# laomao0/BIN

Hardware: AMD Instinct MI355X
Metric: interpolated frames/sec at 1280x720 (higher is better)
Workload: dtype f16x3 (fp16 hi+lo pairs = 22-bit significands, 3 MFMA products, f32 accumulate; fp32-class: 1e-6 vs the fp32 reference); 1 GPU; Adobe240 test_blur 1280x720 inference, batch=1 per GPU (6-frame window padded to 768x1344 by the test.py rule), window-sharded; precision=f16x3, streams=1, pipelined_steps=False, four_call_schedule=False, parity=max-abs <= 2e-5 (f16x3) vs the fp32 reference (tests/)

## Files before the change

bin_amd/csrc/binhip_conv_common.h:

```cpp
#pragma once
#include "binhip_internal.h"
#include <type_traits>
#ifndef BINHIP_TIMELINE
#define BINHIP_TIMELINE 0
#endif

typedef _Float16 half8 __attribute__((ext_vector_type(8)));
typedef _Float16 half4 __attribute__((ext_vector_type(4)));
typedef float floatx16 __attribute__((ext_vector_type(16)));
typedef float floatx4 __attribute__((ext_vector_type(4)));
typedef __attribute__((address_space(3))) void lds_void_t;
typedef unsigned u32x4 __attribute__((ext_vector_type(4)));

int bh_launch_upnet_ring(const void* x_hi, const void* x_lo, const float* wvar, const float* bvar, float* out, const float* const* images,
                         int nimg, int N, int H, int W, int cin, hipStream_t s);
int bh_upnet_gsub(const float* g, int N, int H, int W, const float* scale, void* y_hi, void* y_lo, void* status, hipStream_t s);
int bh_upnet_ring_dgrad(const float* g, const float* wvar, const float* scale, void* gx_hi, void* gx_lo, void* status, int N, int H, int W,
                        int cin, hipStream_t s);
int bh_upnet_ring_wgrad(const float* g, const void* x_hi, const void* x_lo, float* dwvar, float* dbvar, int N, int H, int W, int cin,
                        int accumulate, hipStream_t s);
struct ConvKArgs {
    const _Float16* x_hi;
    const _Float16* x_lo;
    const _Float16* w_hi;
    const _Float16* w_lo;
    const float* bias;
    _Float16* y_hi;
    _Float16* y_lo;
    const _Float16* r_hi;
    const _Float16* r_lo;
    const _Float16* r2_hi;
    const _Float16* r2_lo;
    const _Float16* m_hi;
    float* out_f32;
    const float* img[5];
    unsigned* flags;
    long long group_stride;
    int N, H, W;
// ... 559 lines not shown
```

bin_amd/csrc/binhip_fused.h:

```cpp
#pragma once
#include "binhip_conv_common.h"

struct TailKArgs {
    const _Float16 *x_hi, *x_lo;
    const _Float16 *wc_hi, *wc_lo;
    const _Float16 *wl_hi, *wl_lo;
    const float *bc, *bl;
    _Float16 *y_hi, *y_lo;
    _Float16 *o3_hi, *o3_lo;
    unsigned* flags;
    int N, H, W, tiles_x, tiles_y, wt;
#if BINHIP_TIMELINE
    void* tl;
    unsigned tl_launch, tl_base;
#endif
};

int bh_launch_tail_x3(const TailKArgs& a, hipStream_t s);
```

bin_amd/csrc/binhip_fused.hip:

```cpp
#include "binhip_conv_common.h"

#include "binhip_fused.h"

template <int NT, int NBUF>
struct TailCfg {
    static constexpr int R = 2, NW = 8, TH = 16, PH = 18, PW = 34;
    static constexpr int PP = 20, CWP = 9, LWP = 3;
    static constexpr int NPL = (NT == 3) ? 2 : 1;
    static constexpr int PLANE_BYTES = (PP + CWP + LWP) * 1024;
    static constexpr int BUF_BYTES = NPL * PLANE_BYTES;
    static constexpr int TAILW_BYTES = NPL * 2 * LWP * 1024;
    static constexpr int LDS_BYTES = NBUF * BUF_BYTES + TAILW_BYTES + 1024;
    static constexpr int NPJ = 3, NCJ = 2, NLJ = 1;
    static constexpr int PS = NPL * (NPJ + NCJ + NLJ);
    static constexpr int NCHUNK = 12;
    static_assert(LDS_BYTES <= 160 * 1024, "LDS budget");
    static_assert(NBUF <= 2 || (NBUF - 2) * PS <= 63, "vmcnt immediate range");
    static_assert(NW * R * 32 * 2 * 32 * NPL <= BUF_BYTES, "o3 staging tile must fit one stage buffer");
};

template <class C>
__device__ __forceinline__ void tail_issue(const TailKArgs& a, char* smem, int c, int buf, int wave, int lane,
                                           const unsigned (&voff)[C::NPJ], const ConvTile& t) {
    char* dummy = smem + (C::LDS_BYTES - 1024);
#pragma unroll
    for (int pl = 0; pl < C::NPL; ++pl) {
        char* lds = smem + buf * C::BUF_BYTES + pl * C::PLANE_BYTES;
// ... 4 lines not shown
            const bool real = i < C::PP;
            __builtin_amdgcn_raw_ptr_buffer_load_lds(rs, (lds_void_t*)(real ? lds + i * 1024 : dummy), 16,
                                                     real ? voff[j] : 0x80000000u, 0, 0, 0);
        }
        __amdgpu_buffer_rsrc_t ws = __builtin_amdgcn_make_buffer_rsrc(
            (void*)((pl ? a.wc_lo : a.wc_hi) + (long long)c * (9 * 32 * 16)), 0, 9 * 1024, 0x00020000);
#pragma unroll
        for (int j = 0; j < C::NCJ; ++j) {
            const int i = wave + C::NW * j;
            const bool real = i < C::CWP;
            __builtin_amdgcn_raw_ptr_buffer_load_lds(ws, (lds_void_t*)(real ? lds + (C::PP + i) * 1024 : dummy), 16,
                                                     real ? (unsigned)(lane * 16) : 0x80000000u, real ? i * 1024 : 0, 0, 0);
        }
        __amdgpu_buffer_rsrc_t ls = __builtin_amdgcn_make_buffer_rsrc(
            (void*)((pl ? a.wl_lo : a.wl_hi) + (long long)c * (96 * 16)), 0, 3 * 1024, 0x00020000);
        {
            const bool real = wave < C::LWP;
            __builtin_amdgcn_raw_ptr_buffer_load_lds(ls, (lds_void_t*)(real ? lds + (C::PP + C::CWP + wave) * 1024 : dummy), 16,
                                                     real ? (unsigned)(lane * 16) : 0x80000000u, real ? wave * 1024 : 0, 0, 0);
        }
    }
}

template <int NT, int NBUF>
__global__ void __launch_bounds__(512)
rdb_tail_kernel(const TailKArgs a, const float* __restrict__ bias_c, const float* __restrict__ bias_l) {
    using C = TailCfg<NT, NBUF>;
    extern __shared__ __attribute__((aligned(16))) char smem[];
    const int tid = threadIdx.x;
    const int lane = tid & 63;
    const int wave = __builtin_amdgcn_readfirstlane(tid >> 6);
    const int n = lane & 31, kg = lane >> 5;

    const ConvTile t = tile_decode<C::TH>(a, 1);
    const int img = t.img, tx0 = t.tx0, ty0 = t.ty0;
    const int H = a.H, W = a.W;
    const long long plane_elems = t.plane_elems;

    unsigned voff[C::NPJ];
#pragma unroll
    for (int j = 0; j < C::NPJ; ++j) {
        const int i = wave + C::NW * j;
        const int q = i * 64 + lane;
        const int p = q >> 1, s = q & 1;
        const int py = p / C::PW, px = p - py * C::PW;
        const int gy = ty0 + py - 1, gx = tx0 + px - 1;
        const int cg = s ^ ((p >> 3) & 1);
        const bool ok = (p < C::PH * C::PW) && gy >= 0 && gy < H && gx >= 0 && gx < W;
        voff[j] = ok ? (unsigned)((((long long)img * H + gy) * W + gx) * 32 + cg * 16) : 0x80000000u;
    }
// ... 48 lines not shown
#pragma unroll
            for (int rr = 0; rr < C::R + 2; ++rr) {
                const int p = b_lane_p + rr * C::PW + dx;
                const int off = p * 32 + ((kg ^ ((p >> 3) & 1)) << 4);
                Bh[rr] = ld8(pb + off);
                if constexpr (NT == 3) Bl[rr] = ld8(pb + C::PLANE_BYTES + off);
            }
#pragma unroll
            for (int dy = 0; dy < 3; ++dy) {
                const int off = ((dy * 3 + dx) * 32) * 32 + a_lane_off;
                const half8 Ah = ld8(wb + off);
                half8 Al;
                if constexpr (NT == 3) Al = ld8(wb + C::PLANE_BYTES + off);
#pragma unroll
                for (int r = 0; r < C::R; ++r) {
                    if constexpr (NT == 3) {
                        accc[r] = mfma_32x32x16(Al, Bh[r + dy], accc[r]);
                        accc[r] = mfma_32x32x16(Ah, Bl[r + dy], accc[r]);
                    }
                    accc[r] = mfma_32x32x16(Ah, Bh[r + dy], accc[r]);
                }
            }
            if (dx == 1) {
                if (st < 6) {
#pragma unroll
                    for (int r = 0; r < C::R; ++r) {
#pragma unroll
                        for (int mt = 0; mt < 3; ++mt) {
                            if (mt == (st >> 1)) {
                                accl[mt][r] = mfma_32x32x16(ident[st & 1], Bh[r + 1], accl[mt][r]);
                                if constexpr (NT == 3)
                                    accl[mt][r] = mfma_32x32x16(ident[st & 1], Bl[r + 1], accl[mt][r]);
                            }
                        }
                    }
                }
#pragma unroll
                for (int mt = 0; mt < 3; ++mt) {
                    const int off = (mt * 32) * 32 + a_lane_off;
                    const half8 Ah = ld8(lb + off);
                    half8 Al;
                    if constexpr (NT == 3) Al = ld8(lb + C::PLANE_BYTES + off);
#pragma unroll
                    for (int r = 0; r < C::R; ++r) {
                        if constexpr (NT == 3) {
                            accl[mt][r] = mfma_32x32x16(Al, Bh[r + 1], accl[mt][r]);
                            accl[mt][r] = mfma_32x32x16(Ah, Bl[r + 1], accl[mt][r]);
// ... 108 lines not shown
                    split_pair(v[0], v[1], sat, hv[ge].u[0], lv[ge].u[0]);
                    split_pair(v[2], v[3], sat, hv[ge].u[1], lv[ge].u[1]);
                }
#pragma unroll
                for (int k = 0; k < 2; ++k) {
                    auto sw = __builtin_amdgcn_permlane32_swap(hv[0].u[k], hv[1].u[k], false, false);
                    hv[0].u[k] = sw[0]; hv[1].u[k] = sw[1];
                    if constexpr (NT == 3) {
                        auto sl = __builtin_amdgcn_permlane32_swap(lv[0].u[k], lv[1].u[k], false, false);
                        lv[0].u[k] = sl[0]; lv[1].u[k] = sl[1];
                    }
                }
                if (ok) {
                    store16(a.y_hi, o_slot, make_uint4(hv[0].u[0], hv[0].u[1], hv[1].u[0], hv[1].u[1]), a.wt);
                    if constexpr (NT == 3)
                        store16(a.y_lo, o_slot, make_uint4(lv[0].u[0], lv[0].u[1], lv[1].u[0], lv[1].u[1]), a.wt);
                }
            }
        }
    }
    if (a.flags && __builtin_amdgcn_ballot_w64(sat != 0) != 0 && lane == 0) atomicOr(a.flags, BINHIP_FLAG_SATURATED);
}

template <int NT, int NBUF>
static int launch_tail(const TailKArgs& a0, hipStream_t s) {
    using C = TailCfg<NT, NBUF>;
    static std::atomic<unsigned long long> lds_set{0};
    if (int rc = bh_set_max_lds(&rdb_tail_kernel<NT, NBUF>, C::LDS_BYTES, lds_set)) return rc;
    TailKArgs a = a0;
    rdb_tail_kernel<NT, NBUF><<<dim3(set_tiles<C>(a)), dim3(512), C::LDS_BYTES, s>>>(a, a.bc, a.bl);
    BH_CHECK_LAUNCH();
    return 0;
}

extern "C" {

int binhip_rdb_tail_fwd(int N, int H, int W, int nterms, const void* blk_hi, const void* blk_lo, const void* wc_hi,
                        const void* wc_lo, const float* bias_c, const void* wl_hi, const void* wl_lo, const float* bias_l,
                        void* y_hi, void* y_lo, int store_o3, void* status, void* stream) {
    if (!blk_hi || !wc_hi || !wl_hi || !bias_c || !bias_l || !y_hi) return BINHIP_E_ARG;
    if (nterms != 1 && nterms != 3) return BINHIP_E_ARG;
    if (nterms == 3 && (!blk_lo || !wc_lo || !wl_lo || !y_lo)) return BINHIP_E_ARG;
    if (N <= 0 || H <= 0 || W <= 0) return BINHIP_E_SHAPE;
    if ((long long)N * H * W >= (1ll << 26)) return BINHIP_E_SHAPE;
    TailKArgs a;
    a.x_hi = (const _Float16*)blk_hi; a.x_lo = (const _Float16*)blk_lo;
    a.wc_hi = (const _Float16*)wc_hi; a.wc_lo = (const _Float16*)wc_lo;
    a.wl_hi = (const _Float16*)wl_hi; a.wl_lo = (const _Float16*)wl_lo;
    a.bc = bias_c; a.bl = bias_l;
    a.y_hi = (_Float16*)y_hi; a.y_lo = (_Float16*)y_lo;
    const long long plane = (long long)N * H * W * 16;
    a.o3_hi = store_o3 ? (_Float16*)blk_hi + 12 * plane : nullptr;
    a.o3_lo = (store_o3 && nterms == 3) ? (_Float16*)blk_lo + 12 * plane : nullptr;
    a.flags = (unsigned*)status;
    a.N = N; a.H = H; a.W = W; a.tiles_x = a.tiles_y = 0;
    a.wt = (6 * plane * 2 < (1ll << 32) - 64) ? 1 : 0;
    hipStream_t s = (hipStream_t)stream;
    if (nterms == 1) return launch_tail<1, 2>(a, s);
    return bh_launch_tail_x3(a, s);
}

}
```

bin_amd/csrc/binhip_fused_x3.hip:

```cpp
#include "binhip_fused.h"
#include <type_traits>

namespace {

struct TX {
    static constexpr int R = 2, NW = 4, TH = 8, PH = 10, PW = 34;
    static constexpr int PP = (PH * PW * 2 + 63) / 64;
    static constexpr int CWP = 9, LWP = 3;
    static constexpr int PATCH_BYTES = PP * 1024;
    static constexpr int WPL = (CWP + LWP) * 1024;
    static constexpr int WBUF_BYTES = 2 * WPL;
    static constexpr int W_OFF = 2 * PATCH_BYTES;
    static constexpr int LDS_BYTES = W_OFF + 2 * WBUF_BYTES;
    static constexpr int NCHUNK = 12;
    static constexpr int NPJ = (PP + NW - 1) / NW;
    static constexpr int TAILW_OFF = W_OFF;
    static_assert(2 * LDS_BYTES <= 160 * 1024, "two workgroups per CU");
};

__device__ __forceinline__ void tx_issue_patch(const TailKArgs& a, char* smem, int c, int pl, int wave, const unsigned* voff,
                                               const ConvTile& t) {
    __amdgpu_buffer_rsrc_t rs = patch_plane(a, c, pl, t);
    char* lds = smem + pl * TX::PATCH_BYTES;
#pragma unroll
// ... 99 lines not shown
#pragma unroll
                for (int r = 0; r < R; ++r)
                    accc[r] = mfma_32x32x16(Al[s & 1], B[set][r + k], accc[r]);
            }
#pragma unroll
            for (int r = 0; r < R; ++r)
                accc[r] = mfma_32x32x16(Ah[s & 1], B[set][r + k], accc[r]);
        } else {
            if constexpr (HI) {
#pragma unroll
                for (int r = 0; r < R; ++r)
                    accl[k][r] = mfma_32x32x16(Al[s & 1], B[1][r + 1], accl[k][r]);
            }
#pragma unroll
            for (int r = 0; r < R; ++r)
                accl[k][r] = mfma_32x32x16(Ah[s & 1], B[1][r + 1], accl[k][r]);
        }
        __builtin_amdgcn_sched_barrier(0);
    }
#pragma unroll
    for (int r = 0; r < R; ++r) carry[r] = B[1][r + 1];
}

__global__ void __launch_bounds__(256) __attribute__((amdgpu_waves_per_eu(2, 2)))
rdb_tail_x3_kernel(const TailKArgs a, const float* __restrict__ bias_c, const float* __restrict__ bias_l) {
    extern __shared__ __attribute__((aligned(16))) char smem[];
    BH_TL_DECL;
    BH_TL_BEGIN();
    const int tid = threadIdx.x;
    const int lane = tid & 63;
    const int wave = __builtin_amdgcn_readfirstlane(tid >> 6);
    const int n = lane & 31, kg = lane >> 5;

    const ConvTile t = tile_decode<TX::TH>(a, 1);
    const int img = t.img, tx0 = t.tx0, ty0 = t.ty0;
    const int H = a.H, W = a.W;
    const long long plane_elems = t.plane_elems;
    unsigned voff[TX::NPJ];
    patch_offsets<TX, 1>(voff, t, H, W, wave, lane);

    floatx16 accc[TX::R];
    floatx16 accl[3][TX::R];
#pragma unroll
    for (int r = 0; r < TX::R; ++r)
#pragma unroll
        for (int e = 0; e < 16; ++e) {
// ... 7 lines not shown
    tx_issue_weights(a, smem, 0, 0, wave, lane);
    tx_issue_patch(a, smem, 0, 0, wave, voff, t);
    half8 carry[TX::R];
    auto chunk = [&](const int c, auto res_hi, auto res_lo) __attribute__((always_inline)) {
        constexpr int RH = decltype(res_hi)::value, RL = decltype(res_lo)::value;
        const char* wb = smem + TX::W_OFF + (c & 1) * TX::WBUF_BYTES;
        wait_vmcnt<0>();
        __builtin_amdgcn_s_barrier();
        __builtin_amdgcn_sched_barrier(0);
#if BINHIP_TIMELINE
        if (c == 0) BH_TL_STAMP(1);
#endif
        tx_issue_patch(a, smem, c, 1, wave, voff, t);
        if (c + 1 < TX::NCHUNK) tx_issue_weights(a, smem, c + 1, (c + 1) & 1, wave, lane);
        else tx_issue_tailw(a, smem, wave, lane);
        tx_compute<true, RH>(smem, wb, a_lane_off, b_lane_off, accc, accl, carry);
        wait_vmcnt<0>();
        __builtin_amdgcn_s_barrier();
        __builtin_amdgcn_sched_barrier(0);
        if (c + 1 < TX::NCHUNK) tx_issue_patch(a, smem, c + 1, 0, wave, voff, t);
        tx_compute<false, RL>(smem + TX::PATCH_BYTES, wb, a_lane_off, b_lane_off, accc, accl, carry);
    };
    using std::integral_constant;
    chunk(0, integral_constant<int, -1>{}, integral_constant<int, 0>{});
    chunk(1, integral_constant<int, 0>{}, integral_constant<int, 1>{});
    chunk(2, integral_constant<int, 1>{}, integral_constant<int, 2>{});
    chunk(3, integral_constant<int, 2>{}, integral_constant<int, 3>{});
    chunk(4, integral_constant<int, 3>{}, integral_constant<int, 4>{});
    chunk(5, integral_constant<int, 4>{}, integral_constant<int, 5>{});
    chunk(6, integral_constant<int, 5>{}, integral_constant<int, -1>{});
    for (int c = 7; c < TX::NCHUNK; ++c) chunk(c, integral_constant<int, -1>{}, integral_constant<int, -1>{});
    wait_vmcnt<0>();
    __builtin_amdgcn_s_barrier();
    __builtin_amdgcn_sched_barrier(0);

    __builtin_amdgcn_s_setprio(0);
    const int gx = tx0 + n;
    union H4 { half4 h; unsigned u[2]; };
    union H8 { half8 h; unsigned u[4]; };
    unsigned sat = 0;
    half8 Bh[2][TX::R], Bl[2][TX::R];
#pragma unroll
    for (int r = 0; r < TX::R; ++r) {
        const int gy = ty0 + wave * TX::R + r;
        const bool ok = (gy < H) && (gx < W);
#pragma unroll
        for (int gp = 0; gp < 2; ++gp) {
            H4 hv[2], lv[2];
#pragma unroll
            for (int ge = 0; ge < 2; ++ge) {
                const int g = 2 * gp + ge;
                float b8[8];
#pragma unroll
                for (int j = 0; j < 8; ++j) b8[j] = bias_c[8 * g + j];
// ... 34 lines not shown
            for (int r = 0; r < TX::R; ++r) {
                accl[mt][r] = mfma_32x32x16(Al, Bh[t][r], accl[mt][r]);
                accl[mt][r] = mfma_32x32x16(Ah, Bh[t][r], accl[mt][r]);
                accl[mt][r] = mfma_32x32x16(Ah, Bl[t][r], accl[mt][r]);
            }
        }
    }
    if (a.flags && __builtin_amdgcn_ballot_w64(sat != 0) != 0 && lane == 0) atomicOr(a.flags, BINHIP_FLAG_SATURATED);
    BH_TL_STAMP(2);

    ConvKArgs e;
    e.bias = a.bl; e.y_hi = a.y_hi; e.y_lo = a.y_lo;
    e.r_hi = e.r_lo = e.r2_hi = e.r2_lo = e.m_hi = nullptr;
    e.flags = a.flags;
    e.N = a.N; e.H = H; e.W = W;
    e.relu = 0; e.has_res = 0; e.cout = 96; e.wt = a.wt;
    e.och_limit = 6; e.res_chunks = 0; e.mask_from = 0; e.y_cpg = 0; e.y_cpg_inv = 0; e.y_group_stride = 0; e.y_unshuf = 0;
    conv_epilogue<3, TX::R, 3, BINHIP_EPI_PLANES, false>(e, bias_l, accl, img, ty0 + wave * TX::R, tx0, 0, true, n, kg, plane_elems);
    BH_TL_FINISH(a, blockIdx.x);
}

}

int bh_launch_tail_x3(const TailKArgs& a0, hipStream_t s) {
    static std::atomic<unsigned long long> lds_set{0};
    if (int rc = bh_set_max_lds(&rdb_tail_x3_kernel, TX::LDS_BYTES, lds_set)) return rc;
    TailKArgs a = a0;
    const unsigned grid = set_tiles<TX>(a);
#if BINHIP_TIMELINE
    a.tl = bh_tl_reserve(grid, &a.tl_base);
    a.tl_launch = (2u << 24) | (g_bh_tl_serial.fetch_add(1) & 0xFFFFFFu);
#endif
    rdb_tail_x3_kernel<<<dim3(grid), dim3(256), TX::LDS_BYTES, s>>>(a, a.bc, a.bl);
    BH_CHECK_LAUNCH();
    return 0;
}
```

bin_amd/csrc/binhip_plan.hip:

```cpp
#include "binhip_conv_common.h"

namespace {

struct Shp {
    int G0, D, C, G;
    int c0, cg, cb;
    int L;
    bool stage4;
};
bool resolve_shape(const BinRdnShape* s, Shp* o) {
    Shp h;
    const bool dflt = !s || (s->G0 == 0 && s->D == 0 && s->C == 0 && s->G == 0);
    h.G0 = dflt ? 96 : s->G0; h.D = dflt ? 12 : s->D; h.C = dflt ? 4 : s->C; h.G = dflt ? 32 : s->G;
    if (h.G0 < 32 || h.G0 > 256 || h.G0 % 32 || h.G < 32 || h.G > 128 || h.G % 32) return false;
    if (h.C < 1 || h.C > BINHIP_RDN_MAX_CONVS || h.D < 1 || h.D > 20) return false;
    h.c0 = h.G0 / 16; h.cg = h.G / 16; h.cb = h.c0 + h.C * h.cg;
    h.L = 2 + h.D * (h.C + 1) + 4;
    if (h.L > BINHIP_RDN_MAX_LAYERS) return false;
    h.stage4 = (h.G0 == 96 && h.C == 4 && h.G == 32);
    *o = h;
    return true;
}
inline int layer_conv(const Shp& sh, int d, int c) { return 2 + d * (sh.C + 1) + c; }

// ... 106 lines not shown
        if (l.ks == 1 && l.epi == BINHIP_EPI_PLANES && c.d.W > 32 && c.d.W % 32 == 0) { c.d.H *= c.d.W / 32; c.d.W = 32; }
        if (l.layer == 0 && l.ks == 5 && (12 * nin) % 16 >= 1 && (12 * nin) % 16 <= 8) c.d.reserved = BINHIP_CONV_HALF_LAST_CHUNK;
        c.x_hi = A.hi(l.x); c.x_lo = A.lo(l.x);
        c.w_hi = p->w_hi[l.layer]; c.w_lo = p->w_lo[l.layer]; c.bias = p->bias[l.layer];
        c.r_hi = A.hi(l.res); c.r_lo = A.lo(l.res);
        c.y_hi = A.hi(l.y); c.y_lo = A.lo(l.y);
        c.status = p->status; c.prof = p->profiler;
        if (l.epi == BINHIP_EPI_FINAL || l.epi == BINHIP_EPI_FINAL_SUBPIX) {
            c.y_f32 = out; c.d.n_images = nin;
            for (int i = 0; i < nin; ++i) c.images[i] = inputs[i];
        }
        return c;
    };
    auto conv = [&](const Conv& l) -> int { return bh_launch_conv(mk(l), s); };
    const bool rdb3 = (p->reserved & BINHIP_PLAN_RDB3) && nt == 3 && sh.stage4;
    unsigned* sync_words = (unsigned*)(A.base + w.sync);
    const int cus = binhip_device_cus();
    if (rdb3) {
        hipError_t me = hipMemsetAsync(sync_words, 0, (size_t)(32 + 2 * (size_t)w.tiles) * 4, s);
        if (me != hipSuccess) return (int)me;
    }
    const int64_t P = w.P;
    const int G0 = sh.G0, G = sh.G, C = sh.C, D = sh.D, c0 = sh.c0, cg = sh.cg, cb = sh.cb;
    if ((rc = conv({.layer = 0, .ks = 5, .cin_chunks = w.kc0, .cout = G0, .x = w.x0, .y = w.f1}))) return rc;
    if ((rc = conv({.layer = 1, .cin_chunks = c0, .cout = G0, .x = w.f1, .y = w.blk}))) return rc;
    for (int d = 0; d < D; ++d) {
        const Planes b = w.blk.sub((int64_t)d * cb * P), b_next = b.sub(cb * P);
        auto dense = [&](int c) -> Conv {
            return {.layer = layer_conv(sh, d, c), .cin_chunks = c0 + cg * c, .cout = G, .relu = 1, .x = b, .y = b.sub((c0 + cg * c) * P)};
        };
        const bool fuse = sh.stage4 && !(p->reserved & BINHIP_PLAN_NO_FUSE);
        bool done3 = false;
        if (rdb3 && fuse) {
            ConvKArgs ka[3];
            bool ok3 = true;
            for (int c = 0; c < 3 && ok3; ++c) {
                if ((rc = bh_prepare_conv(mk(dense(c)), &ka[c]))) return rc;
                ok3 = ok3 && ka[c].wt;
            }
            if (ok3) {
                rc = bh_launch_rdb3_x3(ka, sync_words + 32, (unsigned)(d + 1), cus, s);
                if (rc == 0) done3 = true;
                else if (rc != BINHIP_E_SHAPE) return rc;
            }
        }
        for (int c = 0; c < (fuse ? C - 1 : C) && !done3; ++c) if ((rc = conv(dense(c)))) return rc;
        if (fuse) {
            const int L3 = layer_conv(sh, d, 3), LF = layer_conv(sh, d, 4);
            if ((rc = binhip_rdb_tail_fwd(N, h, ww, nt, A.hi(b), A.lo(b), p->w_hi[L3], p->w_lo[L3], p->bias[L3], p->w_hi[LF], p->w_lo[LF], p->bias[LF],
                                          A.hi(b_next), A.lo(b_next), (p->reserved & BINHIP_PLAN_KEEP_ACTS) ? 1 : 0, p->status, stream)))
                return rc;
        } else if ((rc = conv({.layer = layer_conv(sh, d, C), .ks = 1, .cin_chunks = cb, .cout = G0, .x = b, .y = b_next, .res = b})))
            return rc;
    }
    const int LG = sh.L - 4;
    if ((rc = conv({.layer = LG, .ks = 1, .cin_chunks = D * c0, .cout = G0, .x = w.blk.sub(cb * P), .x_cpg = c0, .x_group_stride = cb * P, .y = w.g0})))
        return rc;
    if ((rc = conv({.layer = LG + 1, .cin_chunks = c0, .cout = G0, .x = w.g0, .y = w.g1, .res = w.f1}))) return rc;
    const bool fused_up = (p->reserved & BINHIP_PLAN_FUSED_UPNET) &&
                          (!(p->reserved & BINHIP_PLAN_KEEP_ACTS) || (p->reserved & BINHIP_PLAN_FUSED_UPNET_TRAIN)) &&
                          sh.L + 1 < BINHIP_RDN_MAX_LAYERS && p->w_hi[sh.L] && (nt == 1 || p->w_lo[sh.L]) && p->bias[sh.L] &&
                          p->w_hi[sh.L + 1] && p->bias[sh.L + 1];
    const bool fold = (p->reserved & BINHIP_PLAN_UPNET_FOLD) != 0;
    if (fused_up) {
        if ((rc = conv({.layer = sh.L, .ks = 5, .cin_chunks = c0, .cout = 12, .cout_pad = 32, .epi = BINHIP_EPI_FINAL_SUBPIX, .x = w.g1,
                        .reserved = fold ? BINHIP_CONV_UPNET_FOLD : 0})))
            return rc;
        return bh_launch_upnet_ring(A.hi(w.g1), A.lo(w.g1), (const float*)p->w_hi[sh.L + 1], p->bias[sh.L + 1], out, inputs, nin, N, h, ww,
                                    G0, s);
    }
    if ((rc = conv({.layer = LG + 2, .cin_chunks = c0, .cout = 256, .epi = BINHIP_EPI_SHUFFLE, .x = w.g1, .y = w.u}))) return rc;
    return conv({.layer = LG + 3, .cin_chunks = 4, .cout = 3, .cout_pad = 32, .epi = BINHIP_EPI_FINAL, .H = H, .W = W, .x = w.u});
}

}

namespace {

struct Bws {
// ... 242 lines not shown
```

bin_amd/models/archs/RDN.py:

```python
import ctypes as C
import os

import torch
import torch.nn as nn
import torch.nn.init as weight_init

from ... import ops
from ...rdn_plan import RdnWeights, rdn_forward

PRECISIONS = {"f16": 1, "f16x3": 3}


def default_precision():
    p = os.environ.get("BIN_AMD_PRECISION", "f16x3")
    if p not in PRECISIONS:
        raise ValueError(f"BIN_AMD_PRECISION must be one of {sorted(PRECISIONS)}, got {p!r}")
    return p


class _nullctx:
    def __enter__(self):
        return self

    def __exit__(self, *a):
# ... 77 lines not shown
    N_INPUTS = 0

    def __init__(self, G0=64, D=6, C=4, G=32):
        super().__init__()
        from ...rdn_plan import check_shape
        self.shape = check_shape((G0, D, C, G))
        self.G0, self.D, self.C, self.G = G0, D, C, G
        kSize = 3
        self.SFENet1 = nn.Conv2d(12 * self.N_INPUTS, G0, 5, padding=2, stride=1)
        self.SFENet2 = nn.Conv2d(G0, G0, kSize, padding=1, stride=1)
        self.RDBs = nn.ModuleList([RDB(growRate0=G0, growRate=G, nConvLayers=C) for _ in range(D)])
        self.GFF = nn.Sequential(nn.Conv2d(D * G0, G0, 1, padding=0, stride=1),
                                 nn.Conv2d(G0, G0, kSize, padding=1, stride=1))
        self.UPNet = nn.Sequential(nn.Conv2d(G0, 256, kSize, padding=1, stride=1), nn.PixelShuffle(2),
                                   nn.Conv2d(64, 3, kSize, padding=1, stride=1))
        self.precision = None
        from ...autograd import default_backward_precision, default_wgrad_side_stream
        from ...rdn_plan import default_plan_flags
        self.backward_precision = default_backward_precision()
        self._direct_grads = False
        self.allow_f16_training = False
        self.wgrad_side_stream = default_wgrad_side_stream()
        self.plan_flags = default_plan_flags()
        self.profiler = None
        self.bwd_profiler = None
        self.debug_hook = None
        self._wcache = None
        self._wgen = 0

    def direct_param_grads(self, on=True):
        return _DirectParamGrads([self], on)

    def _weights_key(self, nterms):
        params = list(self.parameters())
        return (nterms, str(params[0].device), self._wgen, tuple((p.data_ptr(), p._version) for p in params))

    def invalidate_kernel_weights(self):
        self._wgen += 1

    def kernel_weights(self, nterms):
        key = self._weights_key(nterms)
        if self._wcache is None or self._wcache[0] != key:
            with torch.no_grad():
                self._wcache = (key, RdnWeights(dict(self.named_parameters()), self.N_INPUTS, nterms, shape=self.shape))
        return self._wcache[1]

    def _run(self, *frames):
        if len(frames) != self.N_INPUTS:
            raise TypeError(f"{type(self).__name__}.forward takes {self.N_INPUTS} frames")
        if not all(f.is_cuda for f in frames):
            raise RuntimeError("bin_amd: RDN sub-networks run on a HIP device only (no CPU fallback; see oracle/)")
        with torch.cuda.device(frames[0].device):
            if torch.is_grad_enabled() and (any(f.requires_grad for f in frames) or
                                             any(p.requires_grad for p in self.parameters())):
                from ...autograd import rdn_apply
                return rdn_apply(self, frames)
            nterms = PRECISIONS[self.precision or default_precision()]
            return rdn_forward(self.kernel_weights(nterms), list(frames), flags=self.plan_flags, profiler=self.profiler)


class RDN_residual_interp_2_input(_RDNBase):
    N_INPUTS = 2

    def forward(self, B0, B1):
        return self._run(B0, B1)


class RDN_residual_interp_2_1_input(_RDNBase):
    N_INPUTS = 3

    def forward(self, I0, I1, I2):
        return self._run(I0, I1, I2)


class RDN_residual_interp_4_1_input(_RDNBase):
    N_INPUTS = 5

    def forward(self, B0, B1, B2, B3, B4):
        return self._run(B0, B1, B2, B3, B4)


# ... 34 lines not shown
            I5 = self.model2_2(I4, I4, I6)
            I7 = self.model2_3(I6, I6, I8)
            I4pp = self.model3_1(I3, B3, I3, I5, B5)
            I6pp = self.model3_2(I5, B5, I5, I7, B7)
            I5ppp = self.model4_1(I4, I4, I4pp, I6pp, I6)
        self.I2_prime, self.I4_prime, self.I6_prime, self.I8_prime = I2, I4, I6, I8
        self.I3_prime, self.I5_prime, self.I7_prime = I3, I5, I7
        self.I4_prime_prime, self.I6_prime_prime, self.I5_prime_prime = I4pp, I6pp, I5ppp
        return I2, I4, I6, I8, I3, I5, I7, I4pp, I6pp, I5ppp


class RDN_residual_interp_5_input_ConvLSTM_L(nn.Module):

    def __init__(self, modelType="lstm"):
        super().__init__()
        self.modelType = modelType
        self.clstm_4_prime = ConvLSTMCell(3, 3)
        self.clstm_6_prime = ConvLSTMCell(3, 3)
        self.clstm_8_prime = ConvLSTMCell(3, 3)
        self.clstm_5_prime_prime = ConvLSTMCell(3, 3)
        self.clstm_7_prime_prime = ConvLSTMCell(3, 3)
        self.clstm_6_prime_prime_prime = ConvLSTMCell(3, 3)
        self.model = RDN_residual_interp_5_input(lstm=True, GO=96, D=12)
        self.prev_state = None
        self.hidden_state = None
        self.reuse_schedule = True
        self.precision = None
        self.n_streams = int(os.environ["BIN_AMD_STREAMS"]) if os.environ.get("BIN_AMD_STREAMS") else None
        self.four_calls = os.environ.get("BIN_AMD_FOUR_CALLS", "1") != "0"
        self.four_calls_infer = os.environ.get("BIN_AMD_INFER_FOUR", "auto")
        self._streams = None

    def set_precision(self, precision):
        if precision is not None and precision not in PRECISIONS:
            raise ValueError(f"precision must be one of {sorted(PRECISIONS)}")
        self.precision = precision
        for m in self.modules():
            if isinstance(m, _RDNBase):
                m.precision = precision
        return self

    def rdn_modules(self):
        seen, out = set(), []
        for m in self.modules():
            if isinstance(m, _RDNBase) and id(m) not in seen:
                seen.add(id(m))
# ... 80 lines not shown
def _forward_streams(self, B, stage1_cache=None, input_events=None):
    from ...rdn_plan import rdn_forward, workspace
    from ... import _lib as L
    dev = B[0].device
    main = torch.cuda.current_stream(dev)
    ns = self.resolved_streams()
    if ns == 1:
        streams = [main]
    else:
        if self._streams is None or len(self._streams) != ns or self._streams[0].device != dev:
            self._streams = [torch.cuda.Stream(device=dev) for _ in range(ns)]
        streams = self._streams
    m = self.model
    mods = {1: m.model1_1, 2: m.model2_1, 3: m.model3_1, 4: m.model4_1}
    nterms = {k: PRECISIONS[v.precision or default_precision()] for k, v in mods.items()}
    wkeys = {k: v._weights_key(nterms[k]) for k, v in mods.items()}
    stale = [v._wcache is None or v._wcache[0] != wkeys[k] for k, v in mods.items()]
    relayout_pending = any(stale)
    kw = {k: v.kernel_weights(nterms[k]) for k, v in mods.items()}
    for k, v in mods.items():
        if (v.plan_flags & L.PLAN_FUSED_UPNET) and kw[k].fused_up is None and kw[k]._up_src is not None:
            kw[k].ensure_fused_upnet()
            relayout_pending = True
    lib = L.lib()
    n, _, h, w = B[0].shape
    ready = {}
    mode = getattr(self, "_graph_mode", None)
    if mode == "capture":
        self._call_graphs = []
    pools = {}
    counter = [0]

    def launch(si, fn, ins):
        if ns == 1 and mode is None:
            return fn()
        s = streams[si % len(streams)]
        for t in ins:
            hit = ready.get(id(t))
            if hit is not None and hit[1] is not s:
                s.wait_event(hit[0])
        if mode == "capture":
            g = torch.cuda.CUDAGraph()
            k = si % len(streams)
            if k not in pools:
                pools[k] = torch.cuda.graph_pool_handle()
            pool = pools[k]
# ... 1 lines not shown
                out = fn()
            self._call_graphs.append((g, out))
        elif mode == "replay":
            g, out = self._call_graphs[counter[0]]
            with torch.cuda.stream(s):
                g.replay()
        else:
            with torch.cuda.stream(s):
                out = fn()
        counter[0] += 1
        e = torch.cuda.Event()
        e.record(s)
        for o in (out if isinstance(out, (tuple, list)) else (out,)):
            ready[id(o)] = (e, s)
        return out

    def rdn(si, k, *ins):
        from ...rdn_plan import c_shape
        nb = lib.binhip_rdn_workspace_bytes(n, h, w, len(ins), nterms[k], C.byref(c_shape(mods[k].shape)))

        def fn():
            ws = workspace(nb, dev, key=f"fwd-stream{si % len(streams)}")
            return rdn_forward(kw[k], [t.contiguous().float() for t in ins], ws=ws, flags=mods[k].plan_flags,
                               profiler=mods[k].profiler)
        return launch(si, fn, ins)

    for s in streams:
        for ev in (input_events or ()):
            s.wait_event(ev)
        if s is main:
            continue
        if input_events is None or relayout_pending:
            s.wait_stream(main)
    cells = (self.clstm_4_prime, self.clstm_6_prime, self.clstm_8_prime, self.clstm_5_prime_prime,
             self.clstm_7_prime_prime, self.clstm_6_prime_prime_prime)

    def cell(si, c, x):
        return launch(si, lambda: c(x, None)[0], [x])

    B1, B3, B5, B7, B9, B11 = B

    touched = set()

    def memo(si, k, *ins):
        if stage1_cache is None:
            return rdn(si, k, *ins)
        key = (k, wkeys[k]) + tuple(id(t) for t in ins)
# ... 73 lines not shown
```

bin_amd/rdn_plan.py:

```python
import ctypes as C

import torch

from . import _lib as L
from .ops import ConvWeights, DgradWeights, RdbGatherWeights, _ptr, _stream, _need_cuda, on_device, relayout_batch, status_word

STAGE4_SHAPE = (96, 12, 4, 32)


def check_shape(shape):
    G0, D, C, G = (int(v) for v in shape)
    if G0 % 32 or not 32 <= G0 <= 256 or G % 32 or not 32 <= G <= 128 or not 1 <= C <= L.RDN_MAX_CONVS or not 1 <= D <= 20 \
            or 2 + D * (C + 1) + 4 > L.RDN_MAX_LAYERS:
        raise NotImplementedError(
            f"bin_amd RDN: unsupported configuration G0={G0}, D={D}, C={C}, G={G} (built: G0 and G multiples of 32 with "
            f"32 <= G0 <= 256, G <= 128; 1 <= C <= {L.RDN_MAX_CONVS}; 1 <= D <= 20)")
    return G0, D, C, G


def c_shape(shape):
    s = L.BinRdnShape()
    s.G0, s.D, s.C, s.G = shape
    return s

# ... 38 lines not shown
    g0 = w4.shape[1]
    assert tuple(w4.shape) == (12, g0, 5, 5) and g0 % 16 == 0
    wc = w4.view(12, g0 // 16, 16, 5, 5)
    slab = w4.new_zeros(g0 // 16, 5, 4, 32, 16)
    for i in range(2):
        for j in range(2):
            rows = slice(2 * i + j, 12, 4)
            taps = wc[rows, :, :, i:i + 4, j:j + 4].permute(1, 3, 4, 0, 2)
            slab[:, 0:4, :, rows] = taps
            slab[:, 1:5, :, slice(16 + 2 * i + j, 28, 4)] = taps
    return slab


def folded_upnet_planes(slab):
    w = slab.float()
    hi = w.half()
    lo = (w - hi.float()).half()
    odd = ((torch.arange(32, device=w.device) >> 3) & 1).bool().view(32, 1, 1)

    def swizzle(p):
        p = p.view(*p.shape[:-1], 2, 8)
        return torch.where(odd, p.flip(-2), p).reshape(-1).contiguous()
    return swizzle(hi), swizzle(lo)


_FUSED_MAPS = {}


def _fused_upnet_maps(device):
    key = str(device)
    if key in _FUSED_MAPS:
        return _FUSED_MAPS[key]
    import numpy as np
    tap = -np.ones((2, 2, 5, 3), dtype=np.int64)
    sub = np.zeros((2, 3), dtype=np.int64)
    for i in range(2):
        for dy in range(3):
            oy, ip = divmod(i + dy - 1, 2)
            sub[i, dy] = ip
            for a in range(3):
                tap[i, ip, oy + 1 + a, a] = dy
    keep = np.ones((3, 2, 3), dtype=bool)
    keep[0, 0, 0] = False
    keep[2, 1, 2] = False
    sh = (3, 3, 3, 2, 2, 5, 5, 64, 2, 2, 3, 3)
    ax = {n: k for k, n in enumerate(("vy", "vx", "c", "i", "j", "t", "u", "k", "ip", "jp", "a", "b"))}
# ... 85 lines not shown
        self.n_inputs, self.nterms, self.shape = n_inputs, nterms, check_shape(shape)
        self.layers = []
        items = []
        for i, nm in enumerate(layer_names(self.shape)):
            w, b = params[f"{prefix}{nm}.weight"], params[f"{prefix}{nm}.bias"]
            shuffle = nm == "UPNet.0"
            cin_chunks = None
            if nm == "SFENet1":
                cin_chunks = (12 * n_inputs + 15) // 16
            self.layers.append(ConvWeights(w, b, nterms=nterms, shuffle=shuffle, cin_chunks=cin_chunks, defer=items))
        assert len(self.layers) == 2 + self.shape[1] * (self.shape[2] + 1) + 4
        relayout_batch(items)

        self._dgrad = None
        w0, _, w2, _ = src = tuple(params[f"{prefix}UPNet.{k}.{t}"] for k in (0, 2) for t in ("weight", "bias"))
        fusable = tuple(w0.shape[2:]) == (3, 3) and w0.shape[0] == 256 and tuple(w2.shape) == (3, 64, 3, 3)
        self._up_src = src if fusable else None
        self.fused_up = None
        self.fused_fold = None
        self.fused_w4 = None
        self.fused_train = None
        self.fused_train_w4 = None
        self.fused_graph = None

    def ensure_fused_upnet(self, train=False):
        if self._up_src is None:
            return None
        if train:
            if self.fused_train is None:
                with torch.enable_grad():
                    leaves = [t.detach().float().requires_grad_() for t in self._up_src]
                    Wr, Br = fused_upnet_operator(*leaves)
                self.fused_graph = (leaves, Wr, Br)
                with torch.no_grad():
                    g0 = Wr.shape[3]
                    self.fused_train_w4 = Wr[4].permute(0, 2, 1).reshape(12, g0, 5, 5).contiguous()
                    main = ConvWeights(self.fused_train_w4, Br[4].detach().contiguous(), nterms=self.nterms)
                    self.fused_train = (main, Wr.detach().contiguous(), Br.detach().contiguous())
            return self.fused_train
        if self.fused_up is None:
            with torch.no_grad():
                W, B = fused_upnet_weights(*self._up_src)
                self.fused_w4 = W[4].float().contiguous()
                main = ConvWeights(self.fused_w4, B[4].float().contiguous(), nterms=self.nterms)
                ring_w = W.permute(0, 1, 3, 4, 2).reshape(9, 12, 25, W.shape[2]).float().contiguous()
                if self.nterms == 3:
                    self.fused_fold = folded_upnet_planes(folded_upnet_weights(W[4]))
                self.fused_up = (main, ring_w, B.float().contiguous())
        return self.fused_up

    def fill_plan(self, plan, fused=None, fold=False):
        plan.shape = c_shape(self.shape)
        for i, cw in enumerate(self.layers):
            plan.w_hi[i] = cw.w_hi.data_ptr()
            plan.w_lo[i] = cw.w_lo.data_ptr() if cw.w_lo is not None else None
            plan.bias[i] = cw.bias.data_ptr()
        n = len(self.layers)
        if fused is not None:
            main, ring_w, ring_b = fused
            plan.w_hi[n], plan.bias[n] = main.w_hi.data_ptr(), main.bias.data_ptr()
            plan.w_lo[n] = main.w_lo.data_ptr() if main.w_lo is not None else None
            if fold:
                plan.w_hi[n], plan.w_lo[n] = (t.data_ptr() for t in self.fused_fold)
            plan.w_hi[n + 1], plan.w_lo[n + 1], plan.bias[n + 1] = ring_w.data_ptr(), None, ring_b.data_ptr()

    def dgrad(self, module, nterms=None, fused=False):
        nterms = self.nterms if nterms is None else nterms
        if self._dgrad is None:
            self._dgrad = {}
        key = (nterms, bool(fused))
        if key not in self._dgrad:
            if fused and self.fused_train is None:
                raise RuntimeError("bin_amd: backward of a fused-UPNet forward on weights that never built the training operands")
            with torch.no_grad():
                self._dgrad[key] = RdnDgradWeights(dict(module.named_parameters()), self.n_inputs, nterms, shape=self.shape,
                                                   fused=(self.fused_train_w4, self.fused_train[1]) if fused else None)
        return self._dgrad[key]


class RdnDgradWeights:

    def __init__(self, params, n_inputs, nterms, prefix="", shape=STAGE4_SHAPE, fused=None):
        self.shape = G0, D, C, G = check_shape(shape)
        self.fused_ring_w = None
        names = layer_names(self.shape)
        self._src = fp32 = {nm: params[f"{prefix}{nm}.weight"].detach().contiguous().float() for nm in names}
        blocks = [[fp32[f"RDBs.{d}.convs.{c}.conv.0"] for c in range(C)] for d in range(D)]
# ... 42 lines not shown
    return ws


def release_workspaces(stream=None):
    if stream is None:
        _workspaces.clear()
        return
    for k in [k for k in _workspaces if k[2] == stream.cuda_stream and k[1] == stream.device.index]:
        del _workspaces[k]


import os as _os


def default_plan_flags():
    flags = L.PLAN_RDB3 if _os.environ.get("BIN_AMD_RDB3", "0") == "1" else 0
    if _os.environ.get("BIN_AMD_FUSED_UPNET", "1") != "0":
        flags |= L.PLAN_FUSED_UPNET
        if _os.environ.get("BIN_AMD_UPNET_FOLD", "1") != "0":
            flags |= L.PLAN_UPNET_FOLD
    return flags


def rdn_forward(weights, inputs, out=None, ws=None, flags=0, profiler=None):
    _need_cuda(*inputs)
    with on_device(inputs[0]):
        return _rdn_forward(weights, inputs, out, ws, flags, profiler)


def _rdn_forward(weights, inputs, out, ws, flags, profiler):
    inputs = [t.contiguous().float() for t in inputs]
    n, c, h, w = inputs[0].shape
    assert c == 3 and len(inputs) == weights.n_inputs
    lib = L.lib()
    plan = L.BinRdnPlan()
    plan.N, plan.H, plan.W, plan.n_inputs, plan.nterms = n, h, w, weights.n_inputs, weights.nterms
    plan.reserved = int(flags or 0)
    plan.status = status_word(inputs[0].device).data_ptr()
    plan.profiler = profiler if profiler else None
    fused, fold = None, False
    if plan.reserved & L.PLAN_FUSED_UPNET:
        if plan.reserved & L.PLAN_FUSED_UPNET_TRAIN:
            fused = weights.ensure_fused_upnet(train=True)
        elif not (plan.reserved & L.PLAN_KEEP_ACTS):
            fused = weights.ensure_fused_upnet()
            fold = bool(plan.reserved & L.PLAN_UPNET_FOLD) and fused is not None and weights.fused_fold is not None
    if not fold:
        plan.reserved &= ~L.PLAN_UPNET_FOLD
    weights.fill_plan(plan, fused, fold)
    nbytes = lib.binhip_rdn_workspace_bytes(n, h, w, weights.n_inputs, weights.nterms, C.byref(plan.shape))
    if nbytes == 0:
        raise RuntimeError(f"bin_amd: unsupported RDN shape N={n} H={h} W={w} (H, W must be even)")
    if ws is None:
        ws = workspace(nbytes, inputs[0].device)
    if out is None:
        out = torch.empty((n, 3, h, w), dtype=torch.float32, device=inputs[0].device)
    arr = (C.c_void_p * len(inputs))(*[t.data_ptr() for t in inputs])
    L.check(lib.binhip_rdn_forward(C.byref(plan), arr, _ptr(out), _ptr(ws), ws.numel(), _stream()), "rdn_forward")
    return out
```

Baseline: 16.08 interpolated frames/s.

## Fold last RDB's local fusion and residual into the global feature fusion conv

Folds the final RDB's 1x1 local-feature-fusion conv and its residual add algebraically into the GFF 1x1 conv. The combined matrix is precomputed on the host in double precision. The last RDB tail now emits GFF's contribution from the last two blocks directly, without a residual, so the GFF conv reads only D-2 block groups and adds the folded output as a residual. This removes one block's worth of GFF input reads and some MFMA work in exchange for extra weight setup, a new non-residual kernel variant, and a possible change in rounding.

```diff
diff --git a/bin_amd/csrc/binhip_conv_common.h b/bin_amd/csrc/binhip_conv_common.h
--- a/bin_amd/csrc/binhip_conv_common.h
+++ b/bin_amd/csrc/binhip_conv_common.h
@@ -14,6 +14,9 @@
 
 int bh_launch_upnet_ring(const void* x_hi, const void* x_lo, const float* wvar, const float* bvar, float* out, const float* const* images,
                          int nimg, int N, int H, int W, int cin, hipStream_t s);
+int bh_launch_rdb_tail(int N, int H, int W, int nterms, const void* blk_hi, const void* blk_lo, const void* wc_hi, const void* wc_lo,
+                       const float* bias_c, const void* wl_hi, const void* wl_lo, const float* bias_l, void* y_hi, void* y_lo, int store_o3,
+                       int residual, void* status, void* stream);
 int bh_upnet_gsub(const float* g, int N, int H, int W, const float* scale, void* y_hi, void* y_lo, void* status, hipStream_t s);
 int bh_upnet_ring_dgrad(const float* g, const float* wvar, const float* scale, void* gx_hi, void* gx_lo, void* status, int N, int H, int W,
                         int cin, hipStream_t s);
diff --git a/bin_amd/csrc/binhip_fused.h b/bin_amd/csrc/binhip_fused.h
--- a/bin_amd/csrc/binhip_fused.h
+++ b/bin_amd/csrc/binhip_fused.h
@@ -16,4 +16,4 @@
 #endif
 };
 
-int bh_launch_tail_x3(const TailKArgs& a, hipStream_t s);
+int bh_launch_tail_x3(const TailKArgs& a, bool residual, hipStream_t s);
diff --git a/bin_amd/csrc/binhip_fused.hip b/bin_amd/csrc/binhip_fused.hip
--- a/bin_amd/csrc/binhip_fused.hip
+++ b/bin_amd/csrc/binhip_fused.hip
@@ -2,7 +2,7 @@
 
 #include "binhip_fused.h"
 
-template <int NT, int NBUF>
+template <int NT, int NBUF, bool RESID>
 struct TailCfg {
     static constexpr int R = 2, NW = 8, TH = 16, PH = 18, PW = 34;
     static constexpr int PP = 20, CWP = 9, LWP = 3;
@@ -53,10 +53,10 @@
     }
 }
 
-template <int NT, int NBUF>
+template <int NT, int NBUF, bool RESID>
 __global__ void __launch_bounds__(512)
 rdb_tail_kernel(const TailKArgs a, const float* __restrict__ bias_c, const float* __restrict__ bias_l) {
-    using C = TailCfg<NT, NBUF>;
+    using C = TailCfg<NT, NBUF, RESID>;
     extern __shared__ __attribute__((aligned(16))) char smem[];
     const int tid = threadIdx.x;
     const int lane = tid & 63;
@@ -151,7 +151,7 @@
                 }
             }
             if (dx == 1) {
-                if (st < 6) {
+                if (RESID && st < 6) {
 #pragma unroll
                     for (int r = 0; r < C::R; ++r) {
 #pragma unroll
@@ -306,22 +306,20 @@
     if (a.flags && __builtin_amdgcn_ballot_w64(sat != 0) != 0 && lane == 0) atomicOr(a.flags, BINHIP_FLAG_SATURATED);
 }
 
-template <int NT, int NBUF>
+template <int NT, int NBUF, bool RESID>
 static int launch_tail(const TailKArgs& a0, hipStream_t s) {
-    using C = TailCfg<NT, NBUF>;
+    using C = TailCfg<NT, NBUF, RESID>;
     static std::atomic<unsigned long long> lds_set{0};
-    if (int rc = bh_set_max_lds(&rdb_tail_kernel<NT, NBUF>, C::LDS_BYTES, lds_set)) return rc;
+    if (int rc = bh_set_max_lds(&rdb_tail_kernel<NT, NBUF, RESID>, C::LDS_BYTES, lds_set)) return rc;
     TailKArgs a = a0;
-    rdb_tail_kernel<NT, NBUF><<<dim3(set_tiles<C>(a)), dim3(512), C::LDS_BYTES, s>>>(a, a.bc, a.bl);
+    rdb_tail_kernel<NT, NBUF, RESID><<<dim3(set_tiles<C>(a)), dim3(512), C::LDS_BYTES, s>>>(a, a.bc, a.bl);
     BH_CHECK_LAUNCH();
     return 0;
 }
 
-extern "C" {
-
-int binhip_rdb_tail_fwd(int N, int H, int W, int nterms, const void* blk_hi, const void* blk_lo, const void* wc_hi,
-                        const void* wc_lo, const float* bias_c, const void* wl_hi, const void* wl_lo, const float* bias_l,
-                        void* y_hi, void* y_lo, int store_o3, void* status, void* stream) {
+int bh_launch_rdb_tail(int N, int H, int W, int nterms, const void* blk_hi, const void* blk_lo, const void* wc_hi,
+                       const void* wc_lo, const float* bias_c, const void* wl_hi, const void* wl_lo, const float* bias_l,
+                       void* y_hi, void* y_lo, int store_o3, int residual, void* status, void* stream) {
     if (!blk_hi || !wc_hi || !wl_hi || !bias_c || !bias_l || !y_hi) return BINHIP_E_ARG;
     if (nterms != 1 && nterms != 3) return BINHIP_E_ARG;
     if (nterms == 3 && (!blk_lo || !wc_lo || !wl_lo || !y_lo)) return BINHIP_E_ARG;
@@ -340,8 +338,17 @@
     a.N = N; a.H = H; a.W = W; a.tiles_x = a.tiles_y = 0;
     a.wt = (6 * plane * 2 < (1ll << 32) - 64) ? 1 : 0;
     hipStream_t s = (hipStream_t)stream;
-    if (nterms == 1) return launch_tail<1, 2>(a, s);
-    return bh_launch_tail_x3(a, s);
-}
-
-}
+    if (nterms == 1) return residual ? launch_tail<1, 2, true>(a, s) : launch_tail<1, 2, false>(a, s);
+    return bh_launch_tail_x3(a, residual != 0, s);
+}
+
+extern "C" {
+
+int binhip_rdb_tail_fwd(int N, int H, int W, int nterms, const void* blk_hi, const void* blk_lo, const void* wc_hi,
+                        const void* wc_lo, const float* bias_c, const void* wl_hi, const void* wl_lo, const float* bias_l,
+                        void* y_hi, void* y_lo, int store_o3, void* status, void* stream) {
+    return bh_launch_rdb_tail(N, H, W, nterms, blk_hi, blk_lo, wc_hi, wc_lo, bias_c, wl_hi, wl_lo, bias_l, y_hi, y_lo, store_o3, 1, status,
+                              stream);
+}
+
+}
diff --git a/bin_amd/csrc/binhip_fused_x3.hip b/bin_amd/csrc/binhip_fused_x3.hip
--- a/bin_amd/csrc/binhip_fused_x3.hip
+++ b/bin_amd/csrc/binhip_fused_x3.hip
@@ -145,6 +145,7 @@
     for (int r = 0; r < R; ++r) carry[r] = B[1][r + 1];
 }
 
+template <bool RESID>
 __global__ void __launch_bounds__(256) __attribute__((amdgpu_waves_per_eu(2, 2)))
 rdb_tail_x3_kernel(const TailKArgs a, const float* __restrict__ bias_c, const float* __restrict__ bias_l) {
     extern __shared__ __attribute__((aligned(16))) char smem[];
@@ -198,14 +199,16 @@
         tx_compute<false, RL>(smem + TX::PATCH_BYTES, wb, a_lane_off, b_lane_off, accc, accl, carry);
     };
     using std::integral_constant;
-    chunk(0, integral_constant<int, -1>{}, integral_constant<int, 0>{});
-    chunk(1, integral_constant<int, 0>{}, integral_constant<int, 1>{});
-    chunk(2, integral_constant<int, 1>{}, integral_constant<int, 2>{});
-    chunk(3, integral_constant<int, 2>{}, integral_constant<int, 3>{});
-    chunk(4, integral_constant<int, 3>{}, integral_constant<int, 4>{});
-    chunk(5, integral_constant<int, 4>{}, integral_constant<int, 5>{});
-    chunk(6, integral_constant<int, 5>{}, integral_constant<int, -1>{});
-    for (int c = 7; c < TX::NCHUNK; ++c) chunk(c, integral_constant<int, -1>{}, integral_constant<int, -1>{});
+    if constexpr (RESID) {
+        chunk(0, integral_constant<int, -1>{}, integral_constant<int, 0>{});
+        chunk(1, integral_constant<int, 0>{}, integral_constant<int, 1>{});
+        chunk(2, integral_constant<int, 1>{}, integral_constant<int, 2>{});
+        chunk(3, integral_constant<int, 2>{}, integral_constant<int, 3>{});
+        chunk(4, integral_constant<int, 3>{}, integral_constant<int, 4>{});
+        chunk(5, integral_constant<int, 4>{}, integral_constant<int, 5>{});
+        chunk(6, integral_constant<int, 5>{}, integral_constant<int, -1>{});
+    }
+    for (int c = RESID ? 7 : 0; c < TX::NCHUNK; ++c) chunk(c, integral_constant<int, -1>{}, integral_constant<int, -1>{});
     wait_vmcnt<0>();
     __builtin_amdgcn_s_barrier();
     __builtin_amdgcn_sched_barrier(0);
@@ -286,16 +289,21 @@
 
 }
 
-int bh_launch_tail_x3(const TailKArgs& a0, hipStream_t s) {
+template <bool RESID>
+static int launch_tail_x3(const TailKArgs& a0, hipStream_t s) {
     static std::atomic<unsigned long long> lds_set{0};
-    if (int rc = bh_set_max_lds(&rdb_tail_x3_kernel, TX::LDS_BYTES, lds_set)) return rc;
+    if (int rc = bh_set_max_lds(&rdb_tail_x3_kernel<RESID>, TX::LDS_BYTES, lds_set)) return rc;
     TailKArgs a = a0;
     const unsigned grid = set_tiles<TX>(a);
 #if BINHIP_TIMELINE
     a.tl = bh_tl_reserve(grid, &a.tl_base);
     a.tl_launch = (2u << 24) | (g_bh_tl_serial.fetch_add(1) & 0xFFFFFFu);
 #endif
-    rdb_tail_x3_kernel<<<dim3(grid), dim3(256), TX::LDS_BYTES, s>>>(a, a.bc, a.bl);
+    rdb_tail_x3_kernel<RESID><<<dim3(grid), dim3(256), TX::LDS_BYTES, s>>>(a, a.bc, a.bl);
     BH_CHECK_LAUNCH();
     return 0;
 }
+
+int bh_launch_tail_x3(const TailKArgs& a, bool residual, hipStream_t s) {
+    return residual ? launch_tail_x3<true>(a, s) : launch_tail_x3<false>(a, s);
+}
diff --git a/bin_amd/csrc/binhip_plan.hip b/bin_amd/csrc/binhip_plan.hip
--- a/bin_amd/csrc/binhip_plan.hip
+++ b/bin_amd/csrc/binhip_plan.hip
@@ -1,4 +1,9 @@
 #include "binhip_conv_common.h"
+
+__attribute__((weak)) int bh_launch_rdb_tail(int N, int H, int W, int nterms, const void* blk_hi, const void* blk_lo, const void* wc_hi,
+                                             const void* wc_lo, const float* bias_c, const void* wl_hi, const void* wl_lo,
+                                             const float* bias_l, void* y_hi, void* y_lo, int store_o3, int residual, void* status,
+                                             void* stream);
 
 namespace {
 
@@ -152,6 +157,9 @@
     }
     const int64_t P = w.P;
     const int G0 = sh.G0, G = sh.G, C = sh.C, D = sh.D, c0 = sh.c0, cg = sh.cg, cb = sh.cb;
+    const int LM = sh.L + 2, LGC = sh.L + 3;
+    auto slot_set = [&](int i) { return i < BINHIP_RDN_MAX_LAYERS && p->w_hi[i] && p->bias[i] && (nt == 1 || p->w_lo[i]); };
+    const bool gff_fold = !(p->reserved & BINHIP_PLAN_KEEP_ACTS) && D >= 3 && slot_set(LM);
     if ((rc = conv({.layer = 0, .ks = 5, .cin_chunks = w.kc0, .cout = G0, .x = w.x0, .y = w.f1}))) return rc;
     if ((rc = conv({.layer = 1, .cin_chunks = c0, .cout = G0, .x = w.f1, .y = w.blk}))) return rc;
     for (int d = 0; d < D; ++d) {
@@ -160,6 +168,7 @@
             return {.layer = layer_conv(sh, d, c), .cin_chunks = c0 + cg * c, .cout = G, .relu = 1, .x = b, .y = b.sub((c0 + cg * c) * P)};
         };
         const bool fuse = sh.stage4 && !(p->reserved & BINHIP_PLAN_NO_FUSE);
+        const bool contract = gff_fold && d == D - 1;
         bool done3 = false;
         if (rdb3 && fuse) {
             ConvKArgs ka[3];
@@ -177,14 +186,27 @@
         for (int c = 0; c < (fuse ? C - 1 : C) && !done3; ++c) if ((rc = conv(dense(c)))) return rc;
         if (fuse) {
             const int L3 = layer_conv(sh, d, 3), LF = layer_conv(sh, d, 4);
-            if ((rc = binhip_rdb_tail_fwd(N, h, ww, nt, A.hi(b), A.lo(b), p->w_hi[L3], p->w_lo[L3], p->bias[L3], p->w_hi[LF], p->w_lo[LF], p->bias[LF],
-                                          A.hi(b_next), A.lo(b_next), (p->reserved & BINHIP_PLAN_KEEP_ACTS) ? 1 : 0, p->status, stream)))
+            if (contract) {
+                if (!bh_launch_rdb_tail) return BINHIP_E_ARG;
+                if ((rc = bh_launch_rdb_tail(N, h, ww, nt, A.hi(b), A.lo(b), p->w_hi[L3], p->w_lo[L3], p->bias[L3], p->w_hi[LM], p->w_lo[LM],
+                                             p->bias[LM], A.hi(b_next), A.lo(b_next), 0, 0, p->status, stream)))
+                    return rc;
+            } else if ((rc = binhip_rdb_tail_fwd(N, h, ww, nt, A.hi(b), A.lo(b), p->w_hi[L3], p->w_lo[L3], p->bias[L3], p->w_hi[LF], p->w_lo[LF],
+                                                 p->bias[LF], A.hi(b_next), A.lo(b_next), (p->reserved & BINHIP_PLAN_KEEP_ACTS) ? 1 : 0,
+                                                 p->status, stream)))
                 return rc;
+        } else if (contract) {
+            if ((rc = conv({.layer = LM, .ks = 1, .cin_chunks = cb, .cout = G0, .x = b, .y = b_next}))) return rc;
         } else if ((rc = conv({.layer = layer_conv(sh, d, C), .ks = 1, .cin_chunks = cb, .cout = G0, .x = b, .y = b_next, .res = b})))
             return rc;
     }
     const int LG = sh.L - 4;
-    if ((rc = conv({.layer = LG, .ks = 1, .cin_chunks = D * c0, .cout = G0, .x = w.blk.sub(cb * P), .x_cpg = c0, .x_group_stride = cb * P, .y = w.g0})))
+    if (gff_fold) {
+        if ((rc = conv({.layer = slot_set(LGC) ? LGC : LG, .ks = 1, .cin_chunks = (D - 2) * c0, .cout = G0, .x = w.blk.sub(cb * P), .x_cpg = c0,
+                        .x_group_stride = cb * P, .y = w.g0, .res = w.blk.sub((int64_t)D * cb * P)})))
+            return rc;
+    } else if ((rc = conv({.layer = LG, .ks = 1, .cin_chunks = D * c0, .cout = G0, .x = w.blk.sub(cb * P), .x_cpg = c0, .x_group_stride = cb * P,
+                           .y = w.g0})))
         return rc;
     if ((rc = conv({.layer = LG + 1, .cin_chunks = c0, .cout = G0, .x = w.g0, .y = w.g1, .res = w.f1}))) return rc;
     const bool fused_up = (p->reserved & BINHIP_PLAN_FUSED_UPNET) &&
diff --git a/bin_amd/models/archs/RDN.py b/bin_amd/models/archs/RDN.py
--- a/bin_amd/models/archs/RDN.py
+++ b/bin_amd/models/archs/RDN.py
@@ -123,6 +123,7 @@
         self.allow_f16_training = False
         self.wgrad_side_stream = default_wgrad_side_stream()
         self.plan_flags = default_plan_flags()
+        self.gff_fold = False
         self.profiler = None
         self.bwd_profiler = None
         self.debug_hook = None
@@ -157,7 +158,8 @@
                 from ...autograd import rdn_apply
                 return rdn_apply(self, frames)
             nterms = PRECISIONS[self.precision or default_precision()]
-            return rdn_forward(self.kernel_weights(nterms), list(frames), flags=self.plan_flags, profiler=self.profiler)
+            return rdn_forward(self.kernel_weights(nterms), list(frames), flags=self.plan_flags, profiler=self.profiler,
+                               gff_fold=self.gff_fold)
 
 
 class RDN_residual_interp_2_input(_RDNBase):
@@ -238,6 +240,9 @@
         self.clstm_7_prime_prime = ConvLSTMCell(3, 3)
         self.clstm_6_prime_prime_prime = ConvLSTMCell(3, 3)
         self.model = RDN_residual_interp_5_input(lstm=True, GO=96, D=12)
+        from ...rdn_plan import default_gff_fold
+        for m in self.rdn_modules():
+            m.gff_fold = default_gff_fold()
         self.prev_state = None
         self.hidden_state = None
         self.reuse_schedule = True
@@ -364,6 +369,8 @@
         if (v.plan_flags & L.PLAN_FUSED_UPNET) and kw[k].fused_up is None and kw[k]._up_src is not None:
             kw[k].ensure_fused_upnet()
             relayout_pending = True
+        if v.gff_fold and kw[k].gff_fold is None and kw[k].ensure_gff_fold() is not None:
+            relayout_pending = True
     lib = L.lib()
     n, _, h, w = B[0].shape
     ready = {}
@@ -411,7 +418,7 @@
         def fn():
             ws = workspace(nb, dev, key=f"fwd-stream{si % len(streams)}")
             return rdn_forward(kw[k], [t.contiguous().float() for t in ins], ws=ws, flags=mods[k].plan_flags,
-                               profiler=mods[k].profiler)
+                               profiler=mods[k].profiler, gff_fold=mods[k].gff_fold)
         return launch(si, fn, ins)
 
     for s in streams:
diff --git a/bin_amd/rdn_plan.py b/bin_amd/rdn_plan.py
--- a/bin_amd/rdn_plan.py
+++ b/bin_amd/rdn_plan.py
@@ -84,6 +84,21 @@
         p = p.view(*p.shape[:-1], 2, 8)
         return torch.where(odd, p.flip(-2), p).reshape(-1).contiguous()
     return swizzle(hi), swizzle(lo)
+
+
+def gff_fold_operands(lff_w, lff_b, gff_w, shape):
+    G0, D, C, G = shape
+    if D < 3:
+        return None
+    H, h = lff_w.double().reshape(G0, G0 + C * G), lff_b.double()
+    g = gff_w.double().reshape(G0, D, G0)
+    M = g[:, D - 1] @ H
+    M[:, :G0] += g[:, D - 2] + g[:, D - 1]
+    return M, g[:, D - 1] @ h
+
+
+def default_gff_fold():
+    return _os.environ.get("BIN_AMD_GFF_FOLD", "1") != "0"
 
 
 _FUSED_MAPS = {}
@@ -215,6 +230,26 @@
         self.fused_train = None
         self.fused_train_w4 = None
         self.fused_graph = None
+        D = self.shape[1]
+        self._gff_src = tuple(params[f"{prefix}{nm}"] for nm in (f"RDBs.{D - 1}.LFF.weight", f"RDBs.{D - 1}.LFF.bias", "GFF.0.weight",
+                                                                  "GFF.0.bias")) if D >= 3 else None
+        self.gff_fold = None
+
+    def ensure_gff_fold(self):
+        if self._gff_src is None or len(self.layers) + 3 >= L.RDN_MAX_LAYERS:
+            return None
+        if self.gff_fold is None:
+            with torch.no_grad():
+                G0, D = self.shape[0], self.shape[1]
+                lff_w, lff_b, gff_w, gff_b = self._gff_src
+                M, m = gff_fold_operands(lff_w, lff_b, gff_w, self.shape)
+                lff = ConvWeights(M.float().reshape(G0, -1, 1, 1).contiguous(), m.float().contiguous(), nterms=self.nterms)
+                gff, cut = self.layers[-4], None
+                assert lff.cout_block == self.layers[-5].cout_block and lff.cin_chunks == self.layers[-5].cin_chunks
+                if gff.cout_block != gff.cout_pad:
+                    cut = ConvWeights(gff_w[:, :(D - 2) * G0].contiguous(), gff_b, nterms=self.nterms)
+                self.gff_fold = (lff, cut)
+        return self.gff_fold
 
     def ensure_fused_upnet(self, train=False):
         if self._up_src is None:
@@ -242,7 +277,7 @@
                 self.fused_up = (main, ring_w, B.float().contiguous())
         return self.fused_up
 
-    def fill_plan(self, plan, fused=None, fold=False):
+    def fill_plan(self, plan, fused=None, fold=False, gff_fold=None):
         plan.shape = c_shape(self.shape)
         for i, cw in enumerate(self.layers):
             plan.w_hi[i] = cw.w_hi.data_ptr()
@@ -256,6 +291,11 @@
             if fold:
                 plan.w_hi[n], plan.w_lo[n] = (t.data_ptr() for t in self.fused_fold)
             plan.w_hi[n + 1], plan.w_lo[n + 1], plan.bias[n + 1] = ring_w.data_ptr(), None, ring_b.data_ptr()
+        if gff_fold is not None:
+            for slot, cw in zip((n + 2, n + 3), gff_fold):
+                if cw is not None:
+                    plan.w_hi[slot], plan.bias[slot] = cw.w_hi.data_ptr(), cw.bias.data_ptr()
+                    plan.w_lo[slot] = cw.w_lo.data_ptr() if cw.w_lo is not None else None
 
     def dgrad(self, module, nterms=None, fused=False):
         nterms = self.nterms if nterms is None else nterms
@@ -344,13 +384,13 @@
     return flags
 
 
-def rdn_forward(weights, inputs, out=None, ws=None, flags=0, profiler=None):
+def rdn_forward(weights, inputs, out=None, ws=None, flags=0, profiler=None, gff_fold=False):
     _need_cuda(*inputs)
     with on_device(inputs[0]):
-        return _rdn_forward(weights, inputs, out, ws, flags, profiler)
-
-
-def _rdn_forward(weights, inputs, out, ws, flags, profiler):
+        return _rdn_forward(weights, inputs, out, ws, flags, profiler, gff_fold)
+
+
+def _rdn_forward(weights, inputs, out, ws, flags, profiler, gff_fold=False):
     inputs = [t.contiguous().float() for t in inputs]
     n, c, h, w = inputs[0].shape
     assert c == 3 and len(inputs) == weights.n_inputs
@@ -369,7 +409,8 @@
             fold = bool(plan.reserved & L.PLAN_UPNET_FOLD) and fused is not None and weights.fused_fold is not None
     if not fold:
         plan.reserved &= ~L.PLAN_UPNET_FOLD
-    weights.fill_plan(plan, fused, fold)
+    gff = weights.ensure_gff_fold() if gff_fold and not (plan.reserved & L.PLAN_KEEP_ACTS) else None
+    weights.fill_plan(plan, fused, fold, gff)
     nbytes = lib.binhip_rdn_workspace_bytes(n, h, w, weights.n_inputs, weights.nterms, C.byref(plan.shape))
     if nbytes == 0:
         raise RuntimeError(f"bin_amd: unsupported RDN shape N={n} H={h} W={w} (H, W must be even)")
```

New measurement: 16.22 interpolated frames/s (median of 6 runs). Within noise of the previous version (+0.9%).
